# dmmsjtu-umich/time-opt-ilqr

Hardware: NVIDIA B200
Metric: horizon-selection solves/sec (batched HOP-LQR, quadrotor n=12, N=128) (higher is better)
Workload: dtype f64

## Files before the change

time-opt-ilqr_b200/csrc/hop_select_pipe_body.cuh:

```cuda
#pragma once
#include "hop_select_mma_body.cuh"

namespace hop { namespace mma {

template <int D, int M>
struct PipeConst {
    static constexpr int n = D - 1;
    static constexpr int BASE = (FastConst<D, M>::SIZE + 1) & ~1;
    static constexpr int QRAWT = BASE;
    static constexpr int KQF = QRAWT + n * n;
    static constexpr int KPF = KQF + 256;
    static constexpr int SIZE = KPF + 256;
};

struct PipeSlab {
    static constexpr int LU = 0;
    static constexpr int EV = 0, QE = 16, PE = 32, YQ = 48, YP = 80, DU = 112;
    static constexpr int STAGE = 128;
    static constexpr int BARS = STAGE + 2 * kStage;
    static constexpr int ROWB = (BARS + 2 + 1) & ~1;
    static constexpr int SIZE = ROWB + 2 * 3 * 16;
};
static_assert(PipeSlab::SIZE <= kWarpScratch, "the pipelined body reuses the sequential body's per-warp slab");

template <int D, int M>
HOP_DEVICE void pipe_const_fill(double* cst, int tid, int nthr) {
    using FC = FusedConst<D, M>;
    using XC = FastConst<D, M>;
    using PC = PipeConst<D, M>;
    constexpr int n = D - 1;
    for (int i = tid; i < n * n; i += nthr) cst[PC::QRAWT + (i % n) * n + (i / n)] = cst[FC::QRAW + i];
    for (int i = tid; i < 256; i += nthr) {
        const int e = i >> 5, lane = i & 31;
        const int I = e >> 2, J = (e >> 1) & 1, s = e & 1;
        const int g = lane >> 2, t = lane & 3;
        const int R = 8 * I + rho(g), C = 8 * J + t + 4 * s;
        const bool in = (R < n && C < n);
        cst[PC::KQF + i] = in ? cst[XC::KQ + R * n + C] : 0.0;
        cst[PC::KPF + i] = in ? cst[XC::KP + R * n + C] : 0.0;
    }
}

HOP_DEVICE int hi_word(double p) {
#if defined(__CUDA_ARCH__)
    return __double2hiint(p);
#else
    long long bits;
    static_assert(sizeof(bits) == sizeof(p), "");
    __builtin_memcpy(&bits, &p, 8);
    return (int)(bits >> 32);
#endif
}
HOP_DEVICE bool pivot_bad(double p) { return (unsigned)(hi_word(p) - 1) >= 0x7fefffffu; }

HOP_DEVICE double pivot_rcp3(double p) {
#if defined(__CUDA_ARCH__)
    double r;
    asm("rcp.approx.ftz.f64 %0, %1;" : "=d"(r) : "d"(p));
    const double e = fma(-p, r, 1.0);
    const double t = fma(e, e, e);
    return fma(r, t, r);
#else
    return (p - p == 0.0) ? 1.0 / p : (p - p);
#endif
}

HOP_DEVICE double wrap_pi_fast(double a) {
    const double pi = 3.141592653589793, two_pi = 6.283185307179586;
    const double s = a + pi;
    if (s >= 0.0 && s < two_pi) return s - pi;
    if (s >= two_pi && s < 2.0 * two_pi) return (s - two_pi) - pi;
    return wrap_pi(a);
}

template <int D, int GI, int GS>
HOP_DEVICE void gj_pivot(Mat& a, int tj, const LaneGeo& L, int& signs) {
    const int gj = 2 * tj + GS;
    const double p = simt::shfl(a.v[GI][GI][GS], (gj << 2) | tj, 32);
    signs |= hi_word(p);
    const double rinv = pivot_rcp3(p);
    double pr[2][2], f[2];
#pragma unroll
    for (int J = 0; J < 2; ++J)
#pragma unroll
        for (int s = 0; s < 2; ++s) pr[J][s] = simt::shfl(a.v[GI][J][s], (gj << 2) | L.t, 32);
#pragma unroll
    for (int I = 0; I < 2; ++I) f[I] = simt::shfl(a.v[I][GI][GS], (L.g << 2) | tj, 32) * rinv;
    const bool isrow = (L.g == gj), iscol = (L.t == tj);
    if (iscol) {
        a.v[0][GI][GS] = 0.0;
        a.v[1][GI][GS] = 0.0;
        pr[GI][GS] = 1.0;
    }
    if (isrow) {
#pragma unroll
        for (int J = 0; J < 2; ++J)
#pragma unroll
            for (int s = 0; s < 2; ++s) a.v[GI][J][s] = 0.0;
        f[GI] = -rinv;
    }
    HOP_FOR_ELEMS(I, J, s) a.v[I][J][s] = fma(-f[I], pr[J][s], a.v[I][J][s]);
}

template <int D, int GI, int GS>
HOP_DEVICE void fe_pivot_lower(Mat& a, int tj, const LaneGeo& L, int& signs, double& p) {
    const int gj = 2 * tj + GS;
    p = simt::shfl(a.v[GI][GI][GS], (gj << 2) | tj, 32);
    signs |= hi_word(p);
    if (8 * GI + 4 * GS + tj == D - 1) return;
    const double rinv = pivot_rcp3(p);
    double pr[2][2], f[2];
#pragma unroll
    for (int J = GI; J < 2; ++J)
#pragma unroll
        for (int s = 0; s < 2; ++s)
            pr[J][s] = simt::shfl(a.v[J][GI][GS], ((2 * L.t + s) << 2) | tj, 32);
#pragma unroll
    for (int I = GI; I < 2; ++I) f[I] = simt::shfl(a.v[I][GI][GS], (L.g << 2) | tj, 32) * rinv;
    if (GI == 0) {
#pragma unroll
        for (int s = 0; s < 2; ++s) a.v[0][0][s] = fma(-f[0], pr[0][s], a.v[0][0][s]);
#pragma unroll
        for (int s = 0; s < 2; ++s) a.v[1][0][s] = fma(-f[1], pr[0][s], a.v[1][0][s]);
    }
#pragma unroll
    for (int s = 0; s < 2; ++s) a.v[1][1][s] = fma(-f[1], pr[1][s], a.v[1][1][s]);
}
HOP_DEVICE void st2(double* p, double a, double b) {
#if defined(__CUDA_ARCH__)
    *reinterpret_cast<double2*>(p) = make_double2(a, b);
#else
    p[0] = a; p[1] = b;
#endif
}
HOP_DEVICE void ld2(const double* p, double& a, double& b) {
#if defined(__CUDA_ARCH__)
    const double2 v = *reinterpret_cast<const double2*>(p);
    a = v.x; b = v.y;
#else
    a = p[0]; b = p[1];
#endif
}
HOP_DEVICE double zero_hi_if(double a, bool z) {
#if defined(__CUDA_ARCH__)
    return __hiloint2double(z ? 0 : __double2hiint(a), __double2loint(a));
#else
    unsigned long long bits;
    __builtin_memcpy(&bits, &a, 8);
    if (z) bits &= 0xffffffffull;
    __builtin_memcpy(&a, &bits, 8);
    return a;
#endif
}
template <int GI>
HOP_DEVICE void gjs_store(const Mat& a, double* buf, bool isrow, int t) {
    if (isrow) {
        st2(buf + 4 * t, a.v[GI][0][0], a.v[GI][1][0]);
        st2(buf + 4 * t + 2, a.v[GI][0][1], a.v[GI][1][1]);
    }
}
template <int GI, int GS>
HOP_DEVICE void fes_store(const Mat& a, double* buf, bool iscol, int g) {
    if (iscol) st2(buf + 2 * g, a.v[0][GI][GS], a.v[1][GI][GS]);
}
template <int D, int GI, int GS, bool HIZ = false>
HOP_DEVICE void gjs_apply(Mat& a, int tj, const LaneGeo& L, int& signs, const double* buf, bool isrow, bool iscol) {
    double pr[2][2], f[2];
    ld2(buf + 4 * L.t, pr[0][0], pr[1][0]);
    ld2(buf + 4 * L.t + 2, pr[0][1], pr[1][1]);
    ld2(buf + 2 * L.g, f[0], f[1]);
    const double p = buf[4 * tj + 2 * GS + GI];
    signs |= ~hi_word(p);
    const double rinv = pivot_rcp3(p);
    f[0] *= rinv;
    f[1] *= rinv;
    if (iscol) {
        a.v[0][GI][GS] = 0.0;
        a.v[1][GI][GS] = 0.0;
        pr[GI][GS] = -1.0;
    }
    if (HIZ) {
#pragma unroll
        for (int J = 0; J < 2; ++J)
#pragma unroll
            for (int s = 0; s < 2; ++s) a.v[GI][J][s] = zero_hi_if(a.v[GI][J][s], isrow);
        if (isrow) f[GI] = -rinv;
    } else if (isrow) {
#pragma unroll
        for (int J = 0; J < 2; ++J)
#pragma unroll
            for (int s = 0; s < 2; ++s) a.v[GI][J][s] = 0.0;
        f[GI] = -rinv;
    }
    HOP_FOR_ELEMS(I, J, s) a.v[I][J][s] = fma(-f[I], pr[J][s], a.v[I][J][s]);
}
template <int D, int GI, int GS>
HOP_DEVICE void fes_apply(Mat& a, int tj, const LaneGeo& L, int& signs, double& p, const double* buf) {
    p = buf[4 * tj + 2 * GS + GI];
    signs |= hi_word(p);
    if (8 * GI + 4 * GS + tj == D - 1) return;
    const double rinv = pivot_rcp3(p);
    double pr[2][2], f[2];
    ld2(buf + 4 * L.t, pr[0][0], pr[1][0]);
    ld2(buf + 4 * L.t + 2, pr[0][1], pr[1][1]);
    ld2(buf + 2 * L.g, f[0], f[1]);
    f[0] *= rinv;
    f[1] *= rinv;
    if (GI == 0) {
#pragma unroll
        for (int s = 0; s < 2; ++s) a.v[0][0][s] = fma(-f[0], pr[0][s], a.v[0][0][s]);
#pragma unroll
        for (int s = 0; s < 2; ++s) a.v[1][0][s] = fma(-f[1], pr[0][s], a.v[1][0][s]);
    }
#pragma unroll
    for (int s = 0; s < 2; ++s) a.v[1][1][s] = fma(-f[1], pr[1][s], a.v[1][1][s]);
}
template <int D, int GI, int GS, int PAR = -1, bool HIZ = false>
HOP_DEVICE void gj3s_round(Mat& a1, Mat& a2, Mat& x, int tj, const LaneGeo& L, int& signs, double& p, double* rowb) {
    const int gj = 2 * tj + GS;
    const bool isrow = (L.g == gj), iscol = (L.t == tj);
    double* buf = rowb + (PAR < 0 ? (tj & 1) : PAR) * 48;
    gjs_store<GI>(a1, buf, isrow, L.t);
    gjs_store<GI>(a2, buf + 16, isrow, L.t);
    fes_store<GI, GS>(x, buf + 32, iscol, L.g);
    simt::sync();
    gjs_apply<D, GI, GS, HIZ>(a1, tj, L, signs, buf, isrow, iscol);
    gjs_apply<D, GI, GS, HIZ>(a2, tj, L, signs, buf + 16, isrow, iscol);
    fes_apply<D, GI, GS>(x, tj, L, signs, p, buf + 32);
}
template <int D, int GI, int GS, bool UNROLL, bool U2 = false>
HOP_DEVICE void gj3s_group(Mat& a1, Mat& a2, Mat& x, const LaneGeo& L, int& signs, double& p, double* rowb) {
    constexpr int first = 8 * GI + 4 * GS;
    constexpr int cnt = (D - first) < 4 ? (D - first) : 4;
    if (UNROLL) {
#pragma unroll
        for (int tj = 0; tj < cnt; ++tj) gj3s_round<D, GI, GS>(a1, a2, x, tj, L, signs, p, rowb);
    } else if (U2) {
#pragma unroll 1
        for (int tj = 0; tj + 1 < cnt; tj += 2) {
            gj3s_round<D, GI, GS, 0, true>(a1, a2, x, tj, L, signs, p, rowb);
            gj3s_round<D, GI, GS, 1, true>(a1, a2, x, tj + 1, L, signs, p, rowb);
        }
        if (cnt & 1) gj3s_round<D, GI, GS, 0, true>(a1, a2, x, cnt - 1, L, signs, p, rowb);
    } else {
#pragma unroll 1
        for (int tj = 0; tj < cnt; ++tj) gj3s_round<D, GI, GS>(a1, a2, x, tj, L, signs, p, rowb);
    }
}

template <int D, int GI, int GS, bool UNROLL>
HOP_DEVICE void gj3_group(Mat& a1, Mat& a2, Mat& x, const LaneGeo& L, int& signs, double& p) {
    constexpr int first = 8 * GI + 4 * GS;
    constexpr int cnt = (D - first) < 4 ? (D - first) : 4;
    if (UNROLL) {
#pragma unroll
        for (int tj = 0; tj < cnt; ++tj) {
            gj_pivot<D, GI, GS>(a1, tj, L, signs);
            gj_pivot<D, GI, GS>(a2, tj, L, signs);
            fe_pivot_lower<D, GI, GS>(x, tj, L, signs, p);
        }
    } else {
#pragma unroll 1
        for (int tj = 0; tj < cnt; ++tj) {
            gj_pivot<D, GI, GS>(a1, tj, L, signs);
            gj_pivot<D, GI, GS>(a2, tj, L, signs);
            fe_pivot_lower<D, GI, GS>(x, tj, L, signs, p);
        }
    }
}
static_assert(rho_inv(0) == 0 && rho_inv(1) == 2 && rho_inv(4) == 1 && rho_inv(7) == 7, "rho_inv(t + 4s) == 2t + s");

template <int KB, bool ACC>
HOP_DEVICE void mma_nt_lower(Mat& Dm, const Mat& X, const Mat& Z) {
    if (!ACC) {
#pragma unroll
        for (int I = 0; I < 2; ++I)
#pragma unroll
            for (int J = 0; J <= I; ++J) { Dm.v[I][J][0] = 0.0; Dm.v[I][J][1] = 0.0; }
    }
#pragma unroll
    for (int kb = 0; kb < KB; ++kb)
#pragma unroll
        for (int I = 0; I < 2; ++I)
#pragma unroll
            for (int J = 0; J <= I; ++J)
                simt::dmma(Dm.v[I][J][0], Dm.v[I][J][1], X.v[I][kb >> 1][kb & 1], Z.v[J][kb >> 1][kb & 1]);
}

template <int D>
struct LastCol {
    static constexpr int k = D - 1, Jk = k >> 3, sk = (k & 7) >> 2, tk = k & 3;
    static constexpr bool split = (D % 4) == 1;
};
template <int D>
HOP_DEVICE void last_col_rows(double (&r)[2], const Mat& M, const LaneGeo& L) {
    using LC = LastCol<D>;
#pragma unroll
    for (int I = 0; I < 2; ++I) r[I] = simt::shfl(M.v[I][LC::Jk][LC::sk], (L.g << 2) | LC::tk, 32);
}
template <int D>
HOP_DEVICE void last_col_cols(double (&c)[2][2], const Mat& M, const LaneGeo& L) {
    using LC = LastCol<D>;
#pragma unroll
    for (int J = 0; J < 2; ++J)
#pragma unroll
        for (int s = 0; s < 2; ++s) c[J][s] = simt::shfl(M.v[J][LC::Jk][LC::sk], ((2 * L.t + s) << 2) | LC::tk, 32);
}
template <bool LOWER>
HOP_DEVICE void rank1_add(Mat& Dm, const double (&r)[2], const double (&c)[2][2]) {
#pragma unroll
    for (int I = 0; I < 2; ++I)
#pragma unroll
        for (int J = 0; J < 2; ++J)
            if (!LOWER || J <= I) {
#pragma unroll
                for (int s = 0; s < 2; ++s) Dm.v[I][J][s] = fma(r[I], c[J][s], Dm.v[I][J][s]);
            }
}


template <int D, int M, int SCHED>
HOP_DEVICE bool select_fused_pipe_body(const FusedArgs& p, int b, double* scratch, const double* cst) {
    using FC = FusedConst<D, M>;
    using XC = FastConst<D, M>;
    using PC = PipeConst<D, M>;
    using PS = PipeSlab;
    constexpr int n = D - 1;
    constexpr int NT = (D + 7) / 8, KB = (D + 3) / 4, KBM = (M + 3) / 4, NTM = (M + 7) / 8;
    constexpr bool LOOPED = (SCHED != 0), SMX = (SCHED >= 2), U2 = (SCHED == 3);
    double* rowb = scratch + PipeSlab::ROWB;
    constexpr bool R1 = LastCol<D>::split;
    constexpr int KD = R1 ? KB - 1 : KB;
    static_assert(D > 8 && D <= 16 && n <= 16 && M <= 4, "one-problem-per-warp mapping: 9 <= d <= 16, m <= 4");
    if (cst[XC::FLAG] != 0.0) return false;
    LaneGeo L;
    L.init();
    double* EV = scratch + PS::EV;
    double* QE = scratch + PS::QE;
    double* PE = scratch + PS::PE;
    bool bad = false;

    Mat RinvT;
    {
        Mat Rs;
        HOP_FOR_ELEMS(I, J, s) {
            const int R = L.row(I), C = L.col(J, s);
            Rs.v[I][J][s] = ((R < M && C < M) ? cst[FC::RS + R * M + C] : 0.0) + ((R == C && R < M) ? p.jitter : 0.0);
        }
        bad = !gj_attempt<M>(Rs, L);
        mat_transpose(RinvT, Rs, L);
    }
    const int h = L.lane >> 4, li = L.lane & 15;
    const bool isx = li < n;
    const double xg_l = isx ? p.xg[(size_t)b * n + li] : 0.0;
    const bool wrap_l = isx && ((p.wrap_mask >> li) & 1u);
    const double uref_l = (L.lane < M) ? cst[FC::UREF + L.lane] : 0.0;
    const double w = p.w[b];
    const double* mat1 = cst + (h ? FC::PF : PC::QRAWT) + li;
    const double* mat2 = cst + (h ? XC::KP : XC::KQ) + li;
    const double* matc = cst + FC::QRAW + li;
    double* V1 = h ? PE : QE;
    if (L.lane < 16) {
        const double v = (L.lane == n) ? -1.0 : 0.0;
        scratch[PS::YQ + L.lane] = v; scratch[PS::YQ + 16 + L.lane] = v;
        scratch[PS::YP + L.lane] = v; scratch[PS::YP + 16 + L.lane] = v;
    }
    const double* KF1 = cst + PC::KQF + L.lane;
    const double* KF2 = cst + PC::KPF + L.lane;

    const size_t baseN = (size_t)b * p.N;
    const double* Xb = p.X + (size_t)b * (p.N + 1) * n;
    const double* Ub = p.U + (size_t)b * p.u_stride;
    static_assert(n * n + n * M + n <= kStage, "staging buffer too small");
    static_assert((n * n) % 2 == 0 && (n * M) % 2 == 0 && n % 2 == 0, "bulk copies need 16-byte multiples");
    double* stage0 = scratch + PS::STAGE;
    unsigned long long* bars = reinterpret_cast<unsigned long long*>(scratch + PS::BARS);
    constexpr int oA = 0, oB = n * n, oR = oB + n * M;
    auto issue = [&](int s) {
        double* st = stage0 + (s & 1) * kStage;
        unsigned long long* bar = bars + (s & 1);
        const unsigned bytes = 8u * (n * n + n * M + (p.a_resid ? n : 0));
        simt::mbar_expect_tx(bar, bytes);
        simt::bulk_g2s(st + oA, p.A + (baseN + s) * n * n, 8u * n * n, bar);
        simt::bulk_g2s(st + oB, p.Bm + (baseN + s) * n * M, 8u * n * M, bar);
        if (p.a_resid) simt::bulk_g2s(st + oR, p.a_resid + (baseN + s) * n, 8u * n, bar);
    };
    if (L.lane == 0) {
        simt::mbar_init(bars, 1);
        simt::mbar_init(bars + 1, 1);
        simt::mbar_fence_init();
    }
    simt::sync();
    if (L.lane == 0) { issue(0); if (1 < p.T_max) issue(1); }
    simt::sync();
    auto bail = [&](int pending_stage) {
        if (pending_stage >= 0) simt::mbar_wait(bars + (pending_stage & 1), (unsigned)((pending_stage >> 1) & 1));
        simt::sync();
        if (L.lane == 0) { simt::mbar_inval(bars); simt::mbar_inval(bars + 1); }
        simt::sync();
        return false;
    };
    auto load_x = [&](int s) { return (isx && s <= p.T_max) ? Xb[(size_t)s * n + li] : 0.0; };
    auto load_u = [&](int s) { return (L.lane < M && s < p.T_max) ? Ub[(size_t)s * M + L.lane] : 0.0; };

    struct Vec { double ev, v1, corner, qy, ye, rsq, rsp; };
    auto vecA = [&](Vec& V, int s, double xs, double us) {
        double ev = 0.0;
        if (isx) {
            ev = xs - xg_l;
            if (wrap_l) ev = wrap_pi_fast(ev);
            if (h == 0) EV[li] = ev;
        }
        V.ev = ev;
        if (L.lane < M) scratch[PS::DU + (s & 1) * 8 + L.lane] = us - uref_l;
    };
    auto vecB = [&](Vec& V) {
        simt::sync();
        double v1 = 0.0, qc = 0.0;
        if (isx) {
#pragma unroll
            for (int j = 0; j < n; ++j) {
                const double ej = EV[j];
                v1 = fma(mat1[j * n], ej, v1);
                qc = fma(ej, matc[j * n], qc);
            }
            V1[li] = v1;
        }
        V.v1 = v1;
        double r0 = (isx && h == 0) ? qc * V.ev : 0.0;
#pragma unroll
        for (int o = 8; o > 0; o >>= 1) r0 += simt::shfl_xor(r0, o, 32);
        V.corner = simt::shfl(r0, 0, 32) + 2.0 * w + p.rho_reg;
    };
    auto vecC = [&](Vec& V, int s) {
        simt::sync();
        double y = 0.0;
        if (isx) {
#pragma unroll
            for (int j = 0; j < n; ++j) y = fma(mat2[j * n], V1[j], y);
            scratch[(h ? PS::YP : PS::YQ) + (s & 1) * 16 + li] = y;
        }
        double r1 = isx ? (h ? y * V.ev : V.v1 * y) : 0.0;
#pragma unroll
        for (int o = 8; o > 0; o >>= 1) r1 += simt::shfl_xor(r1, o, 32);
        V.qy = simt::shfl(r1, 0, 32);
        V.ye = simt::shfl(r1, 16, 32);
    };
    auto vecD = [&](Vec& V, bool live) {
        const double sigq = (V.corner + p.jitter) - V.qy;
        const double sigp = (p.rho_reg + p.jitter) + p.jitter * V.ye;
        bad = bad || (live && (pivot_bad(sigq) || pivot_bad(sigp)));
        V.rsq = pivot_rcp(sigq);
        V.rsp = pivot_rcp(sigp);
    };
    auto closed_inverse = [&](Mat& E, const double* KF, const double* Y, double rs) {
        double yr[2], yc[2][2];
#pragma unroll
        for (int I = 0; I < 2; ++I) yr[I] = Y[L.row(I)];
#pragma unroll
        for (int J = 0; J < 2; ++J)
#pragma unroll
            for (int s = 0; s < 2; ++s) yc[J][s] = Y[L.col(J, s)];
        HOP_FOR_ELEMS(I, J, s) E.v[I][J][s] = fma(yr[I] * yc[J][s], rs, KF[((I * 2 + J) * 2 + s) * 32]);
    };
    const bool kdiag = (cst[XC::FLAG + 1] != 0.0);
    auto ft_closed = [&](Mat& Ft, const Mat& A, const double* Y, double rs) {
        double yc[2][2], kd[2][2], u[2];
#pragma unroll
        for (int J = 0; J < 2; ++J)
#pragma unroll
            for (int s = 0; s < 2; ++s) {
                const int c = L.col(J, s);
                yc[J][s] = Y[c];
                kd[J][s] = (c < n) ? cst[XC::KQ + c * n + c] : 0.0;
            }
#pragma unroll
        for (int I = 0; I < 2; ++I) {
            double a = 0.0;
#pragma unroll
            for (int J = 0; J < 2; ++J)
#pragma unroll
                for (int s = 0; s < 2; ++s) a = fma(A.v[I][J][s], yc[J][s], a);
            a += simt::shfl_xor(a, 1, 32);
            a += simt::shfl_xor(a, 2, 32);
            u[I] = a * rs;
        }
        HOP_FOR_ELEMS(I, J, s) Ft.v[I][J][s] = fma(u[I], yc[J][s], A.v[I][J][s] * kd[J][s]);
    };
    auto load_AB = [&](const double* stg, const double* DU, Mat& A, Mat& Bm) {
        const double* Ak = stg + oA;
        const double* Bk = stg + oB;
        HOP_FOR_ELEMS(I, J, s) {
            const int R = L.row(I), C = L.col(J, s);
            double a = 0.0;
            if (R < n && C < n) {
                a = Ak[R * n + C];
            } else if (R < n && C == n) {
                double sacc = 0.0;
#pragma unroll
                for (int c = 0; c < M; ++c) sacc = fma(Bk[R * M + c], DU[c], sacc);
                a = (p.a_resid ? stg[oR + R] : 0.0) - sacc;
            } else if (R == n && C == n) {
                a = 1.0;
            }
            A.v[I][J][s] = a;
            Bm.v[I][J][s] = (R < n && C < M) ? Bk[R * M + C] : 0.0;
        }
    };

    Vec V0, V1s;
    vecA(V0, 0, load_x(0), load_u(0)); vecB(V0); vecC(V0, 0); vecD(V0, true);
    simt::sync();
    vecA(V1s, 1, load_x(1), load_u(1)); vecB(V1s); vecC(V1s, 1); vecD(V1s, true);
    simt::sync();
    double rsq = V1s.rsq, rsp = V1s.rsp;
    double xcur = load_x(2), ucur = load_u(2);
    PrefixL<D> P;
    simt::mbar_wait(bars + 0, 0u);
    {
        Mat E, A, Bm, Ft, G;
        closed_inverse(E, KF1, scratch + PS::YQ, V0.rsq);
        load_AB(stage0, scratch + PS::DU, A, Bm);
        mma_nt<NT, NT, KB, false>(Ft, A, E);
        mma_nt<NT, NT, KB, false>(G, Ft, A);
        Mat BR;
        mma_nt<NT, NTM, KBM, false>(BR, Bm, RinvT);
        mma_nt<NT, NT, KBM, true>(G, BR, Bm);
        mat_sym(G, L);
        mma_nt<NT, NT, KB, false>(P.fb, E, A);
        mat_copy(P.eb, E);
        mat_copy(P.gb, G);
    }
    Mat X0;
    HOP_FOR_ELEMS(I, J, s) X0.v[I][J][s] = (L.row(I) == L.col(J, s)) ? 1.0 : 0.0;
    ArgMin am;
    am.init();

    for (int k = 0; k < p.T_max; ++k) {
        const bool last = (k + 1 == p.T_max);
        const int q1 = (k + 1) & 1;
        const bool do_vec = (k + 2 <= p.T_max);
        simt::sync();
        if (L.lane == 0 && k + 2 < p.T_max) issue(k + 2);
        const double xnext = load_x(k + 3), unext = load_u(k + 3);
        Mat W, Wt;
        {
            closed_inverse(W, KF1, scratch + PS::YQ + q1 * 16, rsq);
            closed_inverse(Wt, KF2, scratch + PS::YP + q1 * 16, rsp);
            HOP_FOR_ELEMS(I, J, s) {
                const double dg = (I == J && L.row(I) == L.col(J, s) && L.row(I) < D) ? p.jitter : 0.0;
                const double s1 = (W.v[I][J][s] + P.gb.v[I][J][s]) + dg;
                const double s2 = (Wt.v[I][J][s] + P.gb.v[I][J][s]) + dg;
                W.v[I][J][s] = SMX ? -s1 : s1;
                Wt.v[I][J][s] = SMX ? -s2 : s2;
                if (I == J) X0.v[I][J][s] += dg;
            }
        }
        Vec V;
        double piv = 0.0;
        static_assert(D > 12, "the phase placement below assumes four pivot groups");
        vecA(V, k + 2, xcur, ucur);
        int signs = 0;
        if (SMX) {
            gj3s_group<D, 0, 0, false, U2>(W, Wt, X0, L, signs, piv, rowb);
            vecB(V);
            gj3s_group<D, 0, 1, false, U2>(W, Wt, X0, L, signs, piv, rowb);
            vecC(V, k + 2);
            gj3s_group<D, 1, 0, false, U2>(W, Wt, X0, L, signs, piv, rowb);
            vecD(V, do_vec);
            gj3s_group<D, 1, 1, false, U2>(W, Wt, X0, L, signs, piv, rowb);
        } else {
            gj3_group<D, 0, 0, !LOOPED>(W, Wt, X0, L, signs, piv);
            vecB(V);
            gj3_group<D, 0, 1, !LOOPED>(W, Wt, X0, L, signs, piv);
            vecC(V, k + 2);
            gj3_group<D, 1, 0, !LOOPED>(W, Wt, X0, L, signs, piv);
            vecD(V, do_vec);
            gj3_group<D, 1, 1, !LOOPED>(W, Wt, X0, L, signs, piv);
        }
        bad = bad || (signs < 0) || pivot_bad(piv);
        if (simt::ballot(bad) != 0u) return bail(k + 2 < p.T_max ? k + 2 : -1);
        if (k > 0 && L.lane == 0) {
            const double Jt = 0.5 / piv;
            p.J_out[(size_t)b * p.T_max + (k - 1)] = Jt;
            if (k >= p.T_min) am.push(Jt, k);
        }
        double fb_r[2], fb_c[2][2];
        if (R1) { last_col_rows<D>(fb_r, P.fb, L); last_col_cols<D>(fb_c, P.fb, L); }
        {
            Mat T3, acc;
            mma_nt<NT, NT, KD, false>(T3, P.fb, Wt);
            if (R1) { double c[2][2]; last_col_cols<D>(c, Wt, L); rank1_add<false>(T3, fb_r, c); }
            mma_nt_lower<KD, false>(acc, T3, P.fb);
            if (R1) { double r[2]; last_col_rows<D>(r, T3, L); rank1_add<true>(acc, r, fb_c); }
#pragma unroll
            for (int I = 0; I < 2; ++I)
#pragma unroll
                for (int J = 0; J <= I; ++J)
#pragma unroll
                    for (int s = 0; s < 2; ++s) X0.v[I][J][s] = P.eb.v[I][J][s] - acc.v[I][J][s];
        }
        if (last) break;
        simt::mbar_wait(bars + q1, (unsigned)(((k + 1) >> 1) & 1));
        {
            Mat A, Bm, Ft, G;
            load_AB(stage0 + q1 * kStage, scratch + PS::DU + q1 * 8, A, Bm);
            double ft_r[2], ft_c[2][2], w_c[2][2];
            if (kdiag) {
                ft_closed(Ft, A, scratch + PS::YQ + q1 * 16, rsq);
            } else {
                Mat E;
                closed_inverse(E, KF1, scratch + PS::YQ + q1 * 16, rsq);
                mma_nt<NT, NT, KD, false>(Ft, A, E);
                if (R1) {
                    double r[2], c[2][2];
                    last_col_rows<D>(r, A, L); last_col_cols<D>(c, E, L);
                    rank1_add<false>(Ft, r, c);
                }
            }
            mma_nt<NT, NT, KD, false>(G, Ft, A);
            if (R1) {
                double c[2][2];
                last_col_rows<D>(ft_r, Ft, L); last_col_cols<D>(ft_c, Ft, L); last_col_cols<D>(c, A, L);
                rank1_add<false>(G, ft_r, c);
            }
            {
                Mat BR;
                mma_nt<NT, NTM, KBM, false>(BR, Bm, RinvT);
                mma_nt<NT, NT, KBM, true>(G, BR, Bm);
            }
            Mat T1, acc;
            mma_nt<NT, NT, KD, false>(T1, P.fb, W);
            if (R1) { last_col_cols<D>(w_c, W, L); rank1_add<false>(T1, fb_r, w_c); }
            double t1_r[2];
            if (R1) last_col_rows<D>(t1_r, T1, L);
            mma_nt<NT, NT, KD, false>(acc, T1, P.fb);
            if (R1) rank1_add<false>(acc, t1_r, fb_c);
            mat_sub(P.eb, P.eb, acc);
            mat_sym(P.eb, L);
            mma_nt<NT, NT, KD, false>(acc, T1, Ft);
            if (R1) rank1_add<false>(acc, t1_r, ft_c);
            mma_nt<NT, NT, KD, false>(T1, Ft, W);
            if (R1) rank1_add<false>(T1, ft_r, w_c);
            mat_copy(P.fb, acc);
            mma_nt<NT, NT, KD, false>(acc, T1, Ft);
            if (R1) { double r[2]; last_col_rows<D>(r, T1, L); rank1_add<false>(acc, r, ft_c); }
            mat_sub(P.gb, G, acc);
            mat_sym(P.gb, L);
        }
        rsq = V.rsq; rsp = V.rsp;
        xcur = xnext; ucur = unext;
    }
    {
        HOP_FOR_ELEMS(I, J, s)
            if (I == J && L.row(I) == L.col(J, s) && L.row(I) < D) X0.v[I][J][s] += p.jitter;
        double piv = 0.0;
        Mat d1, d2;
        HOP_FOR_ELEMS(I, J, s) d1.v[I][J][s] = d2.v[I][J][s] = (L.row(I) == L.col(J, s)) ? (SMX ? -1.0 : 1.0) : 0.0;
        int signs = 0;
        if (SMX) {
            simt::sync();
            gj3s_group<D, 0, 0, false>(d1, d2, X0, L, signs, piv, rowb);
            gj3s_group<D, 0, 1, false>(d1, d2, X0, L, signs, piv, rowb);
            gj3s_group<D, 1, 0, false>(d1, d2, X0, L, signs, piv, rowb);
            gj3s_group<D, 1, 1, false>(d1, d2, X0, L, signs, piv, rowb);
        } else {
            gj3_group<D, 0, 0, false>(d1, d2, X0, L, signs, piv);
            gj3_group<D, 0, 1, false>(d1, d2, X0, L, signs, piv);
            gj3_group<D, 1, 0, false>(d1, d2, X0, L, signs, piv);
            gj3_group<D, 1, 1, false>(d1, d2, X0, L, signs, piv);
        }
        bad = bad || (signs < 0) || pivot_bad(piv);
        if (simt::ballot(bad) != 0u) return bail(-1);
        if (L.lane == 0) {
            const double Jt = 0.5 / piv;
            p.J_out[(size_t)b * p.T_max + (p.T_max - 1)] = Jt;
            if (p.T_max >= p.T_min) am.push(Jt, p.T_max);
            p.T_out[b] = am.idx;
            p.Jstar_out[b] = am.best;
            p.status[b] = 0;
        }
    }
    return true;
}

}}
```

Measured before the change: 1.714 million.

## Process Gauss-Jordan pivots in pairs per warp sync under SCHED 3

```diff
diff --git a/time-opt-ilqr_b200/csrc/hop_select_pipe_body.cuh b/time-opt-ilqr_b200/csrc/hop_select_pipe_body.cuh
--- a/time-opt-ilqr_b200/csrc/hop_select_pipe_body.cuh
+++ b/time-opt-ilqr_b200/csrc/hop_select_pipe_body.cuh
@@ -19,7 +19,8 @@
     static constexpr int STAGE = 128;
     static constexpr int BARS = STAGE + 2 * kStage;
     static constexpr int ROWB = (BARS + 2 + 1) & ~1;
-    static constexpr int SIZE = ROWB + 2 * 3 * 16;
+    static constexpr int ROWP = 3 * 32;
+    static constexpr int SIZE = ROWB + 2 * ROWP;
 };
 static_assert(PipeSlab::SIZE <= kWarpScratch, "the pipelined body reuses the sequential body's per-warp slab");
 
@@ -163,6 +164,31 @@
 HOP_DEVICE void fes_store(const Mat& a, double* buf, bool iscol, int g) {
     if (iscol) st2(buf + 2 * g, a.v[0][GI][GS], a.v[1][GI][GS]);
 }
+template <int GI, int GS, bool HIZ>
+HOP_DEVICE void gjs_core(Mat& a, int& signs, double (&pr)[2][2], double (&f)[2], double p, double rinv, bool isrow, bool iscol) {
+    signs |= ~hi_word(p);
+    f[0] *= rinv;
+    f[1] *= rinv;
+    if (iscol) {
+        a.v[0][GI][GS] = 0.0;
+        a.v[1][GI][GS] = 0.0;
+        pr[GI][GS] = -1.0;
+    }
+    if (HIZ) {
+#pragma unroll
+        for (int J = 0; J < 2; ++J)
+#pragma unroll
+            for (int s = 0; s < 2; ++s) a.v[GI][J][s] = zero_hi_if(a.v[GI][J][s], isrow);
+        if (isrow) f[GI] = -rinv;
+    } else if (isrow) {
+#pragma unroll
+        for (int J = 0; J < 2; ++J)
+#pragma unroll
+            for (int s = 0; s < 2; ++s) a.v[GI][J][s] = 0.0;
+        f[GI] = -rinv;
+    }
+    HOP_FOR_ELEMS(I, J, s) a.v[I][J][s] = fma(-f[I], pr[J][s], a.v[I][J][s]);
+}
 template <int D, int GI, int GS, bool HIZ = false>
 HOP_DEVICE void gjs_apply(Mat& a, int tj, const LaneGeo& L, int& signs, const double* buf, bool isrow, bool iscol) {
     double pr[2][2], f[2];
@@ -170,56 +196,37 @@
     ld2(buf + 4 * L.t + 2, pr[0][1], pr[1][1]);
     ld2(buf + 2 * L.g, f[0], f[1]);
     const double p = buf[4 * tj + 2 * GS + GI];
-    signs |= ~hi_word(p);
-    const double rinv = pivot_rcp3(p);
+    gjs_core<GI, GS, HIZ>(a, signs, pr, f, p, pivot_rcp3(p), isrow, iscol);
+}
+template <int GI>
+HOP_DEVICE void fes_core(Mat& a, const double (&pr)[2][2], double (&f)[2], double rinv) {
     f[0] *= rinv;
     f[1] *= rinv;
-    if (iscol) {
-        a.v[0][GI][GS] = 0.0;
-        a.v[1][GI][GS] = 0.0;
-        pr[GI][GS] = -1.0;
-    }
-    if (HIZ) {
-#pragma unroll
-        for (int J = 0; J < 2; ++J)
-#pragma unroll
-            for (int s = 0; s < 2; ++s) a.v[GI][J][s] = zero_hi_if(a.v[GI][J][s], isrow);
-        if (isrow) f[GI] = -rinv;
-    } else if (isrow) {
-#pragma unroll
-        for (int J = 0; J < 2; ++J)
-#pragma unroll
-            for (int s = 0; s < 2; ++s) a.v[GI][J][s] = 0.0;
-        f[GI] = -rinv;
-    }
-    HOP_FOR_ELEMS(I, J, s) a.v[I][J][s] = fma(-f[I], pr[J][s], a.v[I][J][s]);
+    if (GI == 0) {
+#pragma unroll
+        for (int s = 0; s < 2; ++s) a.v[0][0][s] = fma(-f[0], pr[0][s], a.v[0][0][s]);
+#pragma unroll
+        for (int s = 0; s < 2; ++s) a.v[1][0][s] = fma(-f[1], pr[0][s], a.v[1][0][s]);
+    }
+#pragma unroll
+    for (int s = 0; s < 2; ++s) a.v[1][1][s] = fma(-f[1], pr[1][s], a.v[1][1][s]);
 }
 template <int D, int GI, int GS>
 HOP_DEVICE void fes_apply(Mat& a, int tj, const LaneGeo& L, int& signs, double& p, const double* buf) {
     p = buf[4 * tj + 2 * GS + GI];
     signs |= hi_word(p);
     if (8 * GI + 4 * GS + tj == D - 1) return;
-    const double rinv = pivot_rcp3(p);
     double pr[2][2], f[2];
     ld2(buf + 4 * L.t, pr[0][0], pr[1][0]);
     ld2(buf + 4 * L.t + 2, pr[0][1], pr[1][1]);
     ld2(buf + 2 * L.g, f[0], f[1]);
-    f[0] *= rinv;
-    f[1] *= rinv;
-    if (GI == 0) {
-#pragma unroll
-        for (int s = 0; s < 2; ++s) a.v[0][0][s] = fma(-f[0], pr[0][s], a.v[0][0][s]);
-#pragma unroll
-        for (int s = 0; s < 2; ++s) a.v[1][0][s] = fma(-f[1], pr[0][s], a.v[1][0][s]);
-    }
-#pragma unroll
-    for (int s = 0; s < 2; ++s) a.v[1][1][s] = fma(-f[1], pr[1][s], a.v[1][1][s]);
+    fes_core<GI>(a, pr, f, pivot_rcp3(p));
 }
 template <int D, int GI, int GS, int PAR = -1, bool HIZ = false>
 HOP_DEVICE void gj3s_round(Mat& a1, Mat& a2, Mat& x, int tj, const LaneGeo& L, int& signs, double& p, double* rowb) {
     const int gj = 2 * tj + GS;
     const bool isrow = (L.g == gj), iscol = (L.t == tj);
-    double* buf = rowb + (PAR < 0 ? (tj & 1) : PAR) * 48;
+    double* buf = rowb + (PAR < 0 ? (tj & 1) : PAR) * PipeSlab::ROWP;
     gjs_store<GI>(a1, buf, isrow, L.t);
     gjs_store<GI>(a2, buf + 16, isrow, L.t);
     fes_store<GI, GS>(x, buf + 32, iscol, L.g);
@@ -228,24 +235,115 @@
     gjs_apply<D, GI, GS, HIZ>(a2, tj, L, signs, buf + 16, isrow, iscol);
     fes_apply<D, GI, GS>(x, tj, L, signs, p, buf + 32);
 }
-template <int D, int GI, int GS, bool UNROLL, bool U2 = false>
+template <int D, int GI, int GS, bool UNROLL>
 HOP_DEVICE void gj3s_group(Mat& a1, Mat& a2, Mat& x, const LaneGeo& L, int& signs, double& p, double* rowb) {
     constexpr int first = 8 * GI + 4 * GS;
     constexpr int cnt = (D - first) < 4 ? (D - first) : 4;
     if (UNROLL) {
 #pragma unroll
         for (int tj = 0; tj < cnt; ++tj) gj3s_round<D, GI, GS>(a1, a2, x, tj, L, signs, p, rowb);
-    } else if (U2) {
-#pragma unroll 1
-        for (int tj = 0; tj + 1 < cnt; tj += 2) {
-            gj3s_round<D, GI, GS, 0, true>(a1, a2, x, tj, L, signs, p, rowb);
-            gj3s_round<D, GI, GS, 1, true>(a1, a2, x, tj + 1, L, signs, p, rowb);
-        }
-        if (cnt & 1) gj3s_round<D, GI, GS, 0, true>(a1, a2, x, cnt - 1, L, signs, p, rowb);
     } else {
 #pragma unroll 1
         for (int tj = 0; tj < cnt; ++tj) gj3s_round<D, GI, GS>(a1, a2, x, tj, L, signs, p, rowb);
     }
+}
+
+struct PairRows { double r[2][2][2], c[2][2], a, b, d; };
+template <int GI, int GS>
+HOP_DEVICE void pair_load(PairRows& x, const double* buf, int tj, const LaneGeo& L) {
+#pragma unroll
+    for (int m = 0; m < 2; ++m) {
+        ld2(buf + 16 * m + 4 * L.t, x.r[m][0][0], x.r[m][1][0]);
+        ld2(buf + 16 * m + 4 * L.t + 2, x.r[m][0][1], x.r[m][1][1]);
+        ld2(buf + 16 * m + 2 * L.g, x.c[m][0], x.c[m][1]);
+    }
+    const int pj = 4 * tj + 2 * GS + GI;
+    x.a = buf[pj];
+    x.b = buf[pj + 4];
+    x.d = buf[16 + pj + 4];
+}
+template <int GI>
+HOP_DEVICE void gjb_store(const Mat& a, double* buf, bool isrow, bool row1, int t) {
+    if (isrow) {
+        double* r = buf + (row1 ? 16 : 0) + 4 * t;
+        st2(r, a.v[GI][0][0], a.v[GI][1][0]);
+        st2(r + 2, a.v[GI][0][1], a.v[GI][1][1]);
+    }
+}
+template <int GI, int GS>
+HOP_DEVICE void feb_store(const Mat& a, double* buf, bool iscol, bool col1, int g) {
+    if (iscol) st2(buf + (col1 ? 16 : 0) + 2 * g, a.v[0][GI][GS], a.v[1][GI][GS]);
+}
+template <int GI, int GS>
+HOP_DEVICE void gjb_apply(Mat& a, int tj, const LaneGeo& L, int& signs, const double* buf, bool row0, bool row1, bool col0, bool col1) {
+    PairRows x;
+    pair_load<GI, GS>(x, buf, tj, L);
+    const double rinv = pivot_rcp3(x.a);
+    const double l = x.b * rinv;
+    const double p1 = fma(-l, x.b, x.d);
+    double r1[2][2], c1[2];
+#pragma unroll
+    for (int J = 0; J < 2; ++J)
+#pragma unroll
+        for (int s = 0; s < 2; ++s) {
+            const bool cj = (J == GI && s == GS && col0);
+            r1[J][s] = fma(-l, cj ? -1.0 : x.r[0][J][s], cj ? 0.0 : x.r[1][J][s]);
+        }
+#pragma unroll
+    for (int I = 0; I < 2; ++I) {
+        const bool rj = (I == GI && row0);
+        c1[I] = fma(-l, rj ? -1.0 : x.c[0][I], rj ? 0.0 : x.c[1][I]);
+    }
+    gjs_core<GI, GS, true>(a, signs, x.r[0], x.c[0], x.a, rinv, row0, col0);
+    gjs_core<GI, GS, true>(a, signs, r1, c1, p1, pivot_rcp3(p1), row1, col1);
+}
+template <int GI, int GS>
+HOP_DEVICE void feb_apply(Mat& a, int tj, const LaneGeo& L, int& signs, const double* buf) {
+    PairRows x;
+    pair_load<GI, GS>(x, buf, tj, L);
+    signs |= hi_word(x.a);
+    const double rinv = pivot_rcp3(x.a);
+    const double p1 = fma(-(x.b * rinv), x.b, x.d);
+    signs |= hi_word(p1);
+    double r1[2][2], c1[2];
+#pragma unroll
+    for (int J = GI; J < 2; ++J)
+#pragma unroll
+        for (int s = 0; s < 2; ++s) r1[J][s] = fma(-(x.r[0][J][s] * rinv), x.b, x.r[1][J][s]);
+#pragma unroll
+    for (int I = GI; I < 2; ++I) c1[I] = fma(-(x.c[0][I] * rinv), x.b, x.c[1][I]);
+    if (GI == 1) { r1[0][0] = r1[0][1] = c1[0] = 0.0; }
+    fes_core<GI>(a, x.r[0], x.c[0], rinv);
+    fes_core<GI>(a, r1, c1, pivot_rcp3(p1));
+}
+template <int GI, int GS>
+HOP_DEVICE void gj3b_round(Mat& a1, Mat& a2, Mat& x, int tj, const LaneGeo& L, int& signs, double* rowb) {
+    const int gj = 2 * tj + GS;
+    const bool row0 = (L.g == gj), row1 = (L.g == gj + 2), col0 = (L.t == tj), col1 = (L.t == tj + 1);
+    double* buf = rowb + (tj >> 1) * PipeSlab::ROWP;
+    gjb_store<GI>(a1, buf, row0 || row1, row1, L.t);
+    gjb_store<GI>(a2, buf + 32, row0 || row1, row1, L.t);
+    feb_store<GI, GS>(x, buf + 64, col0 || col1, col1, L.g);
+    simt::sync();
+    gjb_apply<GI, GS>(a1, tj, L, signs, buf, row0, row1, col0, col1);
+    gjb_apply<GI, GS>(a2, tj, L, signs, buf + 32, row0, row1, col0, col1);
+    feb_apply<GI, GS>(x, tj, L, signs, buf + 64);
+}
+template <int D, int GI, int GS>
+HOP_DEVICE void gj3b_group(Mat& a1, Mat& a2, Mat& x, const LaneGeo& L, int& signs, double& p, double* rowb) {
+    static_assert(D % 2 == 1, "pivot pairs (j, j+1) with j even: pivot d-1 must be the unpaired last one");
+    constexpr int first = 8 * GI + 4 * GS;
+    constexpr int cnt = (D - first) < 4 ? (D - first) : 4;
+#pragma unroll 1
+    for (int tj = 0; tj + 1 < cnt; tj += 2) gj3b_round<GI, GS>(a1, a2, x, tj, L, signs, rowb);
+    if constexpr ((cnt & 1) != 0) gj3s_round<D, GI, GS, (cnt >> 1) & 1, true>(a1, a2, x, cnt - 1, L, signs, p, rowb);
+}
+template <int D>
+HOP_DEVICE void gj3b_sweep(Mat& a1, Mat& a2, Mat& x, const LaneGeo& L, int& signs, double& p, double* rowb) {
+    gj3b_group<D, 0, 0>(a1, a2, x, L, signs, p, rowb);
+    gj3b_group<D, 0, 1>(a1, a2, x, L, signs, p, rowb);
+    gj3b_group<D, 1, 0>(a1, a2, x, L, signs, p, rowb);
+    gj3b_group<D, 1, 1>(a1, a2, x, L, signs, p, rowb);
 }
 
 template <int D, int GI, int GS, bool UNROLL>
@@ -327,7 +425,7 @@
     using PS = PipeSlab;
     constexpr int n = D - 1;
     constexpr int NT = (D + 7) / 8, KB = (D + 3) / 4, KBM = (M + 3) / 4, NTM = (M + 7) / 8;
-    constexpr bool LOOPED = (SCHED != 0), SMX = (SCHED >= 2), U2 = (SCHED == 3);
+    constexpr bool LOOPED = (SCHED != 0), SMX = (SCHED >= 2), BLK = (SCHED == 3);
     double* rowb = scratch + PipeSlab::ROWB;
     constexpr bool R1 = LastCol<D>::split;
     constexpr int KD = R1 ? KB - 1 : KB;
@@ -561,14 +659,22 @@
         static_assert(D > 12, "the phase placement below assumes four pivot groups");
         vecA(V, k + 2, xcur, ucur);
         int signs = 0;
-        if (SMX) {
-            gj3s_group<D, 0, 0, false, U2>(W, Wt, X0, L, signs, piv, rowb);
+        if (BLK) {
+            gj3b_group<D, 0, 0>(W, Wt, X0, L, signs, piv, rowb);
             vecB(V);
-            gj3s_group<D, 0, 1, false, U2>(W, Wt, X0, L, signs, piv, rowb);
+            gj3b_group<D, 0, 1>(W, Wt, X0, L, signs, piv, rowb);
             vecC(V, k + 2);
-            gj3s_group<D, 1, 0, false, U2>(W, Wt, X0, L, signs, piv, rowb);
+            gj3b_group<D, 1, 0>(W, Wt, X0, L, signs, piv, rowb);
             vecD(V, do_vec);
-            gj3s_group<D, 1, 1, false, U2>(W, Wt, X0, L, signs, piv, rowb);
+            gj3b_group<D, 1, 1>(W, Wt, X0, L, signs, piv, rowb);
+        } else if (SMX) {
+            gj3s_group<D, 0, 0, false>(W, Wt, X0, L, signs, piv, rowb);
+            vecB(V);
+            gj3s_group<D, 0, 1, false>(W, Wt, X0, L, signs, piv, rowb);
+            vecC(V, k + 2);
+            gj3s_group<D, 1, 0, false>(W, Wt, X0, L, signs, piv, rowb);
+            vecD(V, do_vec);
+            gj3s_group<D, 1, 1, false>(W, Wt, X0, L, signs, piv, rowb);
         } else {
             gj3_group<D, 0, 0, !LOOPED>(W, Wt, X0, L, signs, piv);
             vecB(V);
@@ -658,7 +764,10 @@
         Mat d1, d2;
         HOP_FOR_ELEMS(I, J, s) d1.v[I][J][s] = d2.v[I][J][s] = (L.row(I) == L.col(J, s)) ? (SMX ? -1.0 : 1.0) : 0.0;
         int signs = 0;
-        if (SMX) {
+        if (BLK) {
+            simt::sync();
+            gj3b_sweep<D>(d1, d2, X0, L, signs, piv, rowb);
+        } else if (SMX) {
             simt::sync();
             gj3s_group<D, 0, 0, false>(d1, d2, X0, L, signs, piv, rowb);
             gj3s_group<D, 0, 1, false>(d1, d2, X0, L, signs, piv, rowb);
```

Result: slower. 1.540 million, median of 6 (-10.1%).
